# Prachet-Dev-Singh/DenseCLIP_Vit_multimodal

Hardware: AMD Instinct MI355X
Metric: images/sec (fwd+bwd) ViT-B/16 DenseCLIP @1024x2048 (higher is better)
Workload: dtype bf16

## Files before the change

denseclip_vit_multimodal_amd/_native.py:

```python
import ctypes
import os
import threading

_HERE = os.path.dirname(os.path.abspath(__file__))
LIB_PATH = os.environ.get("DCLIP_LIB", os.path.join(_HERE, "libdclip.so"))

F32, F16, BF16 = 0, 1, 2
EPI_STORE, EPI_GELU, EPI_RESIDUAL, EPI_GELU_BWD, EPI_SPLITK, EPI_STORE_SCALED = 0, 1, 2, 3, 4, 5
OPT_ATTN_FWD_WAVES, OPT_ATTN_DQ_WAVES, OPT_ATTN_DKDV_WAVES, OPT_GEMM_TILE, OPT_GEMM_TN_TILE = 0, 1, 2, 3, 4
OPT_ATTN_DKDV_QS, OPT_ATTN_FWD_KERNEL, OPT_ATTN_BWD_KERNEL, OPT_ATTN_BWD_BLOCK, OPT_GEMM_TN_COLSUM = 5, 6, 7, 8, 9
OPT_GEMM_EPI, OPT_GEMM_TAIL, OPT_ATTN_FP8_QK, OPT_ATTN_DQ_ISSUE, OPT_ATTN_DQ_ROWS = 10, 11, 12, 13, 14
OPT_ATTN_DQ_DEFER, OPT_GEMM_SCHED, OPT_GEMM_KLOOP = 15, 16, 17
OPT_ATTN_DQ_REDUCE = 18
OPT_ATTN_PREP_ORDER = 19
OPT_ATTN_DQ_DEFER = 15

_c_void_p = ctypes.c_void_p
_i32 = ctypes.c_int
_i64 = ctypes.c_int64
_f32 = ctypes.c_float

_SIGS = {
    "dclip_layernorm_fwd": [_c_void_p, _i32, _c_void_p, _c_void_p, _c_void_p, _i32, _c_void_p, _c_void_p,
                            _i64, _i64, _f32, _c_void_p],
    "dclip_layernorm_bwd": [_c_void_p, _i32, _c_void_p, _i32, _c_void_p, _c_void_p, _c_void_p, _c_void_p, _i32,
                            _c_void_p, _c_void_p, _i64, _i64, _c_void_p],
    "dclip_layernorm_bwd_res": [_c_void_p, _i32, _c_void_p, _i64, _c_void_p, _i32, _c_void_p, _c_void_p, _c_void_p,
                                _c_void_p, _c_void_p, _c_void_p, _i32, _c_void_p, _c_void_p, _c_void_p, _i64, _i64,
                                _c_void_p],
    "dclip_layernorm_bwd_ws_floats": [_i64, _i64],
    "dclip_layernorm_bwd_add": [_c_void_p, _i32, _c_void_p, _c_void_p, _c_void_p, _c_void_p, _c_void_p, _c_void_p,
                                _i32, _c_void_p, _c_void_p, _i32, _c_void_p, _c_void_p, _c_void_p, _i64, _i64,
                                _c_void_p],
    "dclip_layernorm_bwd_scaled_add": [_c_void_p, _i32, _c_void_p, _c_void_p, _c_void_p, _c_void_p, _c_void_p,
                                       _c_void_p, _c_void_p, _i32, _c_void_p, _i32, _c_void_p, _c_void_p, _c_void_p,
                                       _c_void_p, _c_void_p, _i64, _i64, _f32, _c_void_p, _i32, _c_void_p, _c_void_p],
    "dclip_gemm": [_i32, _i32, _c_void_p, _i64, _c_void_p, _i64, _i64, _i64, _i64, _i32, _f32, _c_void_p, _c_void_p,
# ... 127 lines not shown
```

denseclip_vit_multimodal_amd/_torch_ops.py:

```python
import os

import torch

_HERE = os.path.dirname(os.path.abspath(__file__))
LIB_PATH = os.environ.get("DCLIP_TORCH_LIB", os.path.join(_HERE, "libdclip_torch.so"))

_loaded = False


def load():
    global _loaded
    if _loaded:
        return torch.ops.dclip
    if not os.path.exists(LIB_PATH):
        raise RuntimeError(f"libdclip_torch.so not found at {LIB_PATH}: build it with "
                           "`make -C denseclip_vit_multimodal_amd/csrc` (the HIP path has no CPU fallback)")
    from . import _native
    bound = os.path.realpath(os.path.join(os.path.dirname(LIB_PATH), "libdclip.so"))
    if os.path.realpath(_native.LIB_PATH) != bound:
        raise RuntimeError(f"DCLIP_LIB ({_native.LIB_PATH}) is not the libdclip.so that {LIB_PATH} binds ({bound}); "
                           "build a matching adapter and point DCLIP_TORCH_LIB at it")
    _native.load()
    torch.ops.load_library(LIB_PATH)
    _register_fakes()
# ... 26 lines not shown
    def _(dy, x, w, mean, rstd, res, add, ntok, dw, db, lp_dtype):
        return _e(*x.shape, like=x, dtype=f32), _e(*x.shape, like=x, dtype=lp_dtype)

    @reg("dclip::gemm")
    def _(A, B, epi, bias, aux, out_dtype, alpha, scale=None):
        return _e(A.shape[0], B.shape[0], like=A, dtype=out_dtype)

    @reg("dclip::gemm_gelu")
    def _(A, B, bias):
        return _e(A.shape[0], B.shape[0], like=A), _e(A.shape[0], B.shape[0], like=A)

    @reg("dclip::gemm_gelu_h")
    def _(A, B, bias):
        return _e(A.shape[0], B.shape[0], like=A)

    @reg("dclip::gemm_residual_lp")
    def _(A, B, bias, aux):
        return _e(A.shape[0], B.shape[0], like=A, dtype=f32), _e(A.shape[0], B.shape[0], like=A)

    @reg("dclip::weight_grad")
    def _(dy, x, alpha, db, scale=None):
        return _e(dy.shape[1], x.shape[1], like=dy, dtype=f32)

    @reg("dclip::gemm_tn")
    def _(A, B):
        return _e(A.shape[1], B.shape[1], like=A, dtype=f32)

    @reg("dclip::cast")
    def _(x, dtype, scale, scale_t=None):
        return _e(*x.shape, like=x, dtype=dtype)

    @reg("dclip::bn_eval")
    def _(x, w, b, running_mean, running_var, eps, relu):
        return torch.empty_like(x, memory_format=torch.channels_last)

    @reg("dclip::row_scale_add")
    def _(x, y, s):
        return torch.empty_like(y)

    @reg("dclip::grad_scale")
    def _(g, target):
        return _e(4, like=g, dtype=f32)

    @reg("dclip::transpose2d")
    def _(x, dtype):
        return _e(x.shape[1], x.shape[0], like=x, dtype=dtype)
# ... 135 lines not shown
```

denseclip_vit_multimodal_amd/csrc/attention.hip:

```cpp
#include <type_traits>

#include "attn_frag.h"

namespace {

typedef int i32x4 __attribute__((ext_vector_type(4)));
template <int ROWS, int NT>
struct TileRegs {
    static constexpr int PER = ROWS * 8 / NT;
    i32x4 v[PER];
};

template <typename T, int ROWS, int NT>
__device__ __forceinline__ void tile_load(TileRegs<ROWS, NT>& R, const T* __restrict__ base, int64_t ld, int r0,
                                          int N) {
#pragma unroll
    for (int i = 0; i < TileRegs<ROWS, NT>::PER; ++i) {
        const int idx = i * NT + threadIdx.x;
        int gr = r0 + (idx >> 3);
        gr = gr < N ? gr : N - 1;
        gr = gr > 0 ? gr : 0;
        R.v[i] = *(const i32x4*)(base + (int64_t)gr * ld + (idx & 7) * 8);
    }
}
// ... 2200 lines not shown
}

template <typename T>
bool bwd2_launch(const void* qkv, const void* o, const void* dout, const float* lse, float* delta, void* dqkv, int B,
                 int N, int H, float scale, hipStream_t st, void* f8ws = nullptr) {
    if (N < 257 || dclip_option(DCLIP_OPT_ATTN_BWD_KERNEL) == 1) return false;
    const bool ragged = (N - 1) % 256 != 0;
    const int bwd_block = f8ws != nullptr ? 0 : dclip_option(DCLIP_OPT_ATTN_BWD_BLOCK);
    if (ragged && (dclip_option(DCLIP_OPT_ATTN_DQ_WAVES) == 4 ||
                   (bwd_block != 0 && bwd_block != 5 && bwd_block != 6 && bwd_block != 7 && bwd_block != 8 &&
                    bwd_block != 9 && bwd_block != 10)))
        return false;
    const int nsplit = (N + R0_CHUNK - 1) / R0_CHUNK;
    float* ws0 = delta + (int64_t)B * H * N;
    float* nstat = ws0 + (int64_t)B * H * ((N + 63) / 64) * 192;
    const bool dq4 = dclip_option(DCLIP_OPT_ATTN_DQ_WAVES) == 4;
    if ((bwd_block == 0 || bwd_block == 9 || bwd_block == 10) && f8ws == nullptr) {
        const int64_t bhn = (int64_t)B * H * N;
        float* ds0v = nstat + 2 * bhn;
        void* part = (void*)(((uintptr_t)(ds0v + bhn) + 255) & ~(uintptr_t)255);
        const int nqp = attn_bwd1_prep_blocks(N), nkb = (N - 1 + 255) / 256;
        float* r0kv = ws0;
        float* r0q = ws0 + (int64_t)B * H * nqp * 128;
        attn_bwd1_launch(std::is_same<T, bf16>::value ? DCLIP_BF16 : DCLIP_F16, qkv, o, dout, lse, delta, nstat, ds0v,
                         r0kv, r0q, part, dqkv, B, N, H, scale, st);
        attn_bwd_row0_fold_merge<T><<<B * H, 64, 0, st>>>((const T*)qkv, (const T*)dout, lse, delta, r0kv, nqp, r0q, nkb,
                                                          (T*)dqkv, N, H, scale, 1.0f / LOG2E);
        return true;
    }
    if (bwd_block == 0 || bwd_block == 6 || bwd_block == 7 || bwd_block == 8) {
        const int nq = (N - 1 + (dq4 ? 127 : 255)) / (dq4 ? 128 : 256), nkb = (N - 1 + 255) / 256;
        float* r0kv = ws0;
        float* r0q = ws0 + (int64_t)B * H * nq * 128;
        if (dq4)
            attn_bwd_dq2_kernel<T, 4><<<B * H * nq, 256, 0, st>>>((const T*)qkv, (const T*)o, (const T*)dout, lse,
                                                                   delta, nstat, (T*)dqkv, N, H, scale, r0kv);
        else if (dclip_option(DCLIP_OPT_ATTN_DQ_DEFER) == 1)
            attn_bwd_dq2_kernel<T, 8, false, 1, true><<<B * H * nq, 512, 0, st>>>((const T*)qkv, (const T*)o,
                                                                                   (const T*)dout, lse, delta, nstat,
                                                                                   (T*)dqkv, N, H, scale, r0kv);
        else if (dclip_option(DCLIP_OPT_ATTN_DQ_ROWS) == 64)
            attn_bwd_dq2_kernel<T, 4, false, 2><<<B * H * nq, 256, 0, st>>>((const T*)qkv, (const T*)o,
                                                                             (const T*)dout, lse, delta, nstat,
                                                                             (T*)dqkv, N, H, scale, r0kv);
        else if (dclip_option(DCLIP_OPT_ATTN_DQ_ISSUE) == 1)
            attn_bwd_dq2_kernel<T, 8, true><<<B * H * nq, 512, 0, st>>>((const T*)qkv, (const T*)o, (const T*)dout,
                                                                         lse, delta, nstat, (T*)dqkv, N, H, scale, r0kv);
        else
            attn_bwd_dq2_kernel<T, 8><<<B * H * nq, 512, 0, st>>>((const T*)qkv, (const T*)o, (const T*)dout, lse,
                                                                   delta, nstat, (T*)dqkv, N, H, scale, r0kv);
// ... 101 lines not shown
extern "C" int64_t dclip_attn_bwd_workspace(int B, int N, int H) {
    const int64_t two_pass = bwd_ws_two_pass(B, N, H);
    if (N >= 257) return two_pass + (int64_t)B * H * N + (attn_bwd1_part_bytes(B, N, H) + 3) / 4 + 64;
    return two_pass;
}

static bool bwd_one_pass(int N) {
    if (N < 257 || dclip_option(DCLIP_OPT_ATTN_BWD_KERNEL) == 1) return false;
    if ((N - 1) % 256 != 0 && dclip_option(DCLIP_OPT_ATTN_DQ_WAVES) == 4) return false;
    const int blk = dclip_option(DCLIP_OPT_ATTN_BWD_BLOCK);
    return blk == 0 || blk == 9 || blk == 10;
}

extern "C" int dclip_attn_bwd(int dt, const void* qkv, const void* o, const void* dout, const float* lse,
                              float* delta_ws, void* dqkv, int B, int N, int H, int D, float scale, void* stream) {
    DCLIP_HOST_CHECK(D == HD, "dclip_attn_bwd: head_dim must be 64 (got %d)", D);
    DCLIP_HOST_CHECK(dt == DCLIP_BF16 || dt == DCLIP_F16, "dclip_attn_bwd: dtype must be f16/bf16");
    DCLIP_HOST_CHECK(B > 0 && N > 0 && H > 0, "dclip_attn_bwd: empty problem");
    DCLIP_HOST_CHECK(!bwd_one_pass(N) ||
                         (1 + 64 * (int64_t)((N - 1 + 63) / 64)) * (int64_t)((N - 1 + 255) / 256) * 128 < (1ll << 32),
                     "dclip_attn_bwd: N too large for the one-pass backward's dQ partials (N = %d; "
                     "DCLIP_OPT_ATTN_BWD_BLOCK 6 selects the two-pass backward)", N);
    hipStream_t st = (hipStream_t)stream;
    if (dt == DCLIP_BF16) bwd_launch<bf16>(qkv, o, dout, lse, delta_ws, dqkv, B, N, H, scale, st);
    else bwd_launch<f16>(qkv, o, dout, lse, delta_ws, dqkv, B, N, H, scale, st);
    DCLIP_LAUNCH_CHECK();
    return 0;
}

extern "C" int64_t dclip_attn_bwd_fp8_workspace(int B, int N, int H) {
    return bwd_ws_two_pass(B, N, H) + (attn_bwd_fp8_ws_bytes(B, N, H) + 3) / 4 + 64;
}

extern "C" int dclip_attn_bwd_fp8(int dt, const void* qkv, const void* o, const void* dout, const float* lse, float* ws,
                                  void* dqkv, int B, int N, int H, int D, float scale, void* stream) {
    DCLIP_HOST_CHECK(D == HD, "dclip_attn_bwd_fp8: head_dim must be 64 (got %d)", D);
    DCLIP_HOST_CHECK(dt == DCLIP_BF16 || dt == DCLIP_F16, "dclip_attn_bwd_fp8: dtype must be f16/bf16");
    DCLIP_HOST_CHECK(B > 0 && N > 0 && H > 0, "dclip_attn_bwd_fp8: empty problem");
    DCLIP_HOST_CHECK(ws != nullptr && ((uintptr_t)ws % 16) == 0, "dclip_attn_bwd_fp8: ws (16-B aligned) required");
    DCLIP_HOST_CHECK((int64_t)((N - 1 + 63) / 64) * (8192 + 256) < (1ll << 32),
                     "dclip_attn_bwd_fp8: N too large for the fp8 image ring");
    hipStream_t st = (hipStream_t)stream;
    const int64_t w16 = bwd_ws_two_pass(B, N, H);
    void* f8 = (void*)(((uintptr_t)(ws + w16) + 255) & ~(uintptr_t)255);
    if (dt == DCLIP_BF16) bwd_launch<bf16>(qkv, o, dout, lse, ws, dqkv, B, N, H, scale, st, f8);
    else bwd_launch<f16>(qkv, o, dout, lse, ws, dqkv, B, N, H, scale, st, f8);
// ... 4 lines not shown
```

denseclip_vit_multimodal_amd/csrc/attention_bwd1.hip:

```cpp
#include "dkdv_frag.h"

namespace {

constexpr int B1_NW = 4, B1_KB = 64 * B1_NW;
typedef Dkv2Ctx<bf16, B1_NW> B1Ring;
constexpr int B1_RING = 4 * B1Ring::SLOT;
constexpr int B1_W0 = B1_RING;
constexpr int B1_SMEM = B1_W0 + B1_KB * 4;
constexpr int B1_IMG = B1_KB * 128;
static_assert(B1_SMEM + 2 * B1_IMG <= 160 * 1024, "LDS");

__device__ __forceinline__ int lane_now() {
    int l;
    asm volatile("v_mbcnt_lo_u32_b32 %0, -1, 0\n\tv_mbcnt_hi_u32_b32 %0, -1, %0" : "=v"(l));
    return l;
}

template <typename F>
__device__ __forceinline__ F to_agpr(F v) {
    F r;
    asm volatile("" : "=a"(r) : "0"(v));
    return r;
}

// ... 821 lines not shown
    for (int e = 0; e < 8; ++e) acc[e] = w * (float)kv[e];
    const T* p = dqpart + ((int64_t)bh * Np + q) * nkb * 64 + c8;
    int j = 0;
    for (; j + 8 <= nkb; j += 8) {
        t8 v[8];
#pragma unroll
        for (int u = 0; u < 8; ++u) v[u] = __builtin_nontemporal_load((const t8*)(p + (j + u) * 64));
#pragma unroll
        for (int u = 0; u < 8; ++u)
#pragma unroll
            for (int e = 0; e < 8; ++e) acc[e] += (float)v[u][e];
    }
    for (; j < nkb; ++j) {
        const t8 v = __builtin_nontemporal_load((const t8*)(p + j * 64));
#pragma unroll
        for (int e = 0; e < 8; ++e) acc[e] += (float)v[e];
    }
    t8 r;
#pragma unroll
    for (int e = 0; e < 8; ++e) r[e] = (T)(unscaled ? acc[e] * sc : acc[e]);
    *(t8*)(dqkv + ((int64_t)b * N + q) * ld + hd * HD + c8) = r;
}

constexpr int RQ_Q = 8;
constexpr int RQ_MAX_NKB = 56;
template <typename T>
__global__ __launch_bounds__(256) void attn_bwd1_dq_reduce_lds(const T* __restrict__ dqpart,
                                                               const float* __restrict__ ds0v,
                                                               const T* __restrict__ qkv, T* __restrict__ dqkv,
                                                               int N, int H, int nkb, int nrb, float sc) {
    typedef T t2 __attribute__((ext_vector_type(2)));
    typedef unsigned u32x4 __attribute__((ext_vector_type(4)));
    extern __shared__ __attribute__((aligned(16))) char rq_lds[];
    const int rb = blockIdx.x % nrb, bh = blockIdx.x / nrb, b = bh / H, hd = bh % H;
    const int q0 = 1 + rb * RQ_Q;
    const int C = H * HD;
    const int64_t ld = 3 * (int64_t)C;
    const int64_t Np = 1 + 64 * (int64_t)((N - 1 + 63) / 64);
    const int run = nkb * 128, stride = run + 128;
    const char* src = (const char*)(dqpart + ((int64_t)bh * Np + q0) * nkb * 64);
    const int chunks = RQ_Q * nkb * 8;
    for (int c = threadIdx.x; c < chunks; c += 256) {
        const int qi = c / (nkb * 8), w = c - qi * (nkb * 8);
        const u32x4 v = __builtin_nontemporal_load((const u32x4*)(src + (int64_t)c * 16));
        *(u32x4*)(rq_lds + qi * stride + w * 16) = v;
    }
// ... 1 lines not shown
    const int qi = threadIdx.x >> 5, cp = threadIdx.x & 31;
    const int q = q0 + qi;
    if (q >= N) return;
    const t2 kv = *(const t2*)(qkv + (int64_t)b * N * ld + C + hd * HD + 2 * cp);
    constexpr bool unscaled = std::is_same<T, bf16>::value;
    const float w = ds0v[(int64_t)bh * N + q] * (unscaled ? 1.0f : sc);
    float a0 = w * (float)kv[0], a1 = w * (float)kv[1];
    const char* row = rq_lds + qi * stride + cp * 4;
#pragma unroll 8
    for (int j = 0; j < nkb; ++j) {
        const t2 v = *(const t2*)(row + j * 128);
        a0 += (float)v[0];
        a1 += (float)v[1];
    }
    const t2 r = {(T)(unscaled ? a0 * sc : a0), (T)(unscaled ? a1 * sc : a1)};
    *(t2*)(dqkv + ((int64_t)b * N + q) * ld + hd * HD + 2 * cp) = r;
}

template <typename T>
void bwd1_launch(const void* qkv, const void* o, const void* dout, const float* lse, float* delta, float* nstat,
                 float* ds0v, float* r0kv, int nqp, float* r0q, void* dqpart, void* dqkv, int B, int N, int H,
                 float scale, hipStream_t st) {
    const int nkb = (N - 1 + B1_KB - 1) / B1_KB;
    attn_bwd1_prep_kernel<T><<<B * H * nqp, 256, 0, st>>>((const T*)qkv, (const T*)o, (const T*)dout, lse, delta, nstat,
                                                          ds0v, r0kv, N, H, nqp,
                                                          dclip_option(DCLIP_OPT_ATTN_PREP_ORDER) == 1);
    if (dclip_option(DCLIP_OPT_ATTN_BWD_BLOCK) != 9)
        attn_bwd1b_kernel<T><<<B * H * nkb, 256, 0, st>>>((const T*)qkv, (const T*)dout, lse, delta, nstat,
                                                          nstat + (int64_t)B * H * N, (T*)dqkv, (T*)dqpart, N, H,
                                                          1.0f / LOG2E, scale, r0q);
    else
        attn_bwd1_kernel<T><<<B * H * nkb, 256, 0, st>>>((const T*)qkv, (const T*)dout, lse, delta, nstat,
                                                         nstat + (int64_t)B * H * N, (T*)dqkv, (T*)dqpart, N, H,
                                                         1.0f / LOG2E, scale, r0q);
    if (dclip_option(DCLIP_OPT_ATTN_DQ_REDUCE) == 1 && nkb <= RQ_MAX_NKB) {
        const int nrb = (N - 1 + RQ_Q - 1) / RQ_Q;
        attn_bwd1_dq_reduce_lds<T><<<B * H * nrb, 256, RQ_Q * (nkb * 128 + 128), st>>>(
            (const T*)dqpart, ds0v, (const T*)qkv, (T*)dqkv, N, H, nkb, nrb, scale / DsScale<T>::v);
        return;
    }
    const int nrb = (N - 1 + 31) / 32;
    attn_bwd1_dq_reduce<T><<<B * H * nrb, 256, 0, st>>>((const T*)dqpart, ds0v, (const T*)qkv, (T*)dqkv, N, H, nkb, nrb,
                                                        scale / DsScale<T>::v);
}

}

int attn_bwd1_prep_blocks(int N) { return (N - 1 + 127) / 128; }

int64_t attn_bwd1_part_bytes(int B, int N, int H) {
    const int64_t nkb = (N - 1 + B1_KB - 1) / B1_KB, np = 1 + 64 * (int64_t)((N - 1 + 63) / 64);
    return (int64_t)B * H * nkb * np * 128;
}

void attn_bwd1_launch(int dt, const void* qkv, const void* o, const void* dout, const float* lse, float* delta,
                      float* nstat, float* ds0v, float* r0kv, float* r0q, void* dqpart, void* dqkv, int B, int N,
                      int H, float scale, hipStream_t st) {
    const int nqp = attn_bwd1_prep_blocks(N);
// ... 6 lines not shown
```

denseclip_vit_multimodal_amd/csrc/torch_ops.cpp:

```cpp
#include <ATen/ATen.h>
#include <c10/core/DeviceGuard.h>
#include <c10/hip/HIPStream.h>
#include <torch/library.h>

#include "../../include/dclip.h"

namespace {

using at::Tensor;

int dt_code(at::ScalarType t) {
    switch (t) {
        case at::kFloat: return DCLIP_F32;
        case at::kHalf: return DCLIP_F16;
        case at::kBFloat16: return DCLIP_BF16;
        default: TORCH_CHECK(false, "dclip: unsupported dtype ", t);
    }
    return -1;
}

void* stream_of(const Tensor& t) { return (void*)c10::hip::getCurrentHIPStream(t.device().index()).stream(); }

void check_gpu(const Tensor& t, const char* what, bool contiguous = true) {
    TORCH_CHECK(t.defined(), "dclip: ", what, " is undefined");
    TORCH_CHECK(t.is_cuda(), "dclip: ", what, " must be a GPU tensor (the MI355X path has no CPU fallback)");
    if (contiguous) TORCH_CHECK(t.is_contiguous(), "dclip: ", what, " must be contiguous");
// ... 193 lines not shown
}

Tensor weight_grad(const Tensor& dy, const Tensor& x, double alpha, c10::optional<Tensor> db,
                   const c10::optional<Tensor>& scale) {
    check_gpu(dy, "dy"); check_gpu(x, "x");
    TORCH_CHECK(dy.dim() == 2 && x.dim() == 2 && dy.size(0) == x.size(0), "weight_grad: dy (M, N), x (M, K)");
    TORCH_CHECK(dy.scalar_type() == x.scalar_type(), "weight_grad: dy and x dtypes differ (", dy.scalar_type(), " vs ",
                x.scalar_type(), ")");
    c10::DeviceGuard g(dy.device());
    const int64_t M = dy.size(0), N = dy.size(1), K = x.size(1);
    check_vec(db, N, "weight_grad db");
    int splits = 0;
    int64_t k_pad = 0;
    DCLIP_CALL(dclip_gemm_tn_plan(N, K, M, &splits, &k_pad));
    Tensor dW = at::empty({N, K}, like(dy, at::kFloat));
    Tensor ws = at::empty({(int64_t)splits * (N * K + N)}, like(dy, at::kFloat));
    DCLIP_CALL(dclip_gemm_tn(DCLIP_EPI_SPLITK, dt_code(dy.scalar_type()), dy.data_ptr(), dy.stride(0), x.data_ptr(),
                             x.stride(0), N, K, M, k_pad, splits, (float)alpha, scale_entry(scale, 1), nullptr, ws.data_ptr(),
                             dW.data_ptr(), K,
                             optr<float>(db), stream_of(dy)));
    return dW;
}

Tensor gemm_tn(const Tensor& A, const Tensor& B) {
    check_gpu(A, "A"); check_gpu(B, "B");
    TORCH_CHECK(A.dim() == 2 && B.dim() == 2 && A.size(0) == B.size(0), "gemm_tn: A (K, M), B (K, N)");
    c10::DeviceGuard g(A.device());
    const int64_t K = A.size(0), M = A.size(1), N = B.size(1);
    Tensor out = at::empty({M, N}, like(A, at::kFloat));
    DCLIP_CALL(dclip_gemm_tn(DCLIP_EPI_STORE, dt_code(A.scalar_type()), A.data_ptr(), A.stride(0), B.data_ptr(),
                             B.stride(0), M, N, K, (K + 63) / 64 * 64, 1, 1.0f, nullptr, nullptr, nullptr, out.data_ptr(), N,
                             nullptr, stream_of(A)));
    return out;
}

Tensor grad_scale(const Tensor& g, double target) {
    check_gpu(g, "g");
    TORCH_CHECK(g.scalar_type() == at::kFloat && g.is_contiguous(), "grad_scale: g must be contiguous f32");
    c10::DeviceGuard gd(g.device());
    Tensor ws = at::zeros({4}, g.options());
    DCLIP_CALL(dclip_grad_scale(ptr<float>(g), g.numel(), (float)target, ptr<float>(ws), stream_of(g)));
    return ws;
}

Tensor cast(const Tensor& x, at::ScalarType dtype, double scale, const c10::optional<Tensor>& scale_t) {
    check_gpu(x, "x");
// ... 173 lines not shown
                              (int)H, 64, (float)scale, stream_of(qkv)));
    return {o, lse};
}

std::tuple<Tensor, Tensor> attn_fwd_fp8(const Tensor& qkv, int64_t B, int64_t N, int64_t H) {
    check_gpu(qkv, "qkv");
    TORCH_CHECK(qkv.dim() == 2 && qkv.size(0) == B * N && qkv.size(1) == 3 * 64 * H, "attn_fwd_fp8: qkv (B*N, 3*H*64)");
    c10::DeviceGuard g(qkv.device());
    Tensor o = at::empty({B * N, 64 * H}, qkv.options());
    Tensor lse = at::empty({B * H * N}, like(qkv, at::kFloat));
    Tensor ws = at::empty({dclip_attn_fwd_fp8_workspace((int)B, (int)N, (int)H)}, like(qkv, at::kByte));
    DCLIP_CALL(dclip_attn_fwd_fp8(dt_code(qkv.scalar_type()), qkv.data_ptr(), o.data_ptr(), ptr<float>(lse), ws.data_ptr(),
                                  (int)B, (int)N, (int)H, 64, stream_of(qkv)));
    return {o, lse};
}

Tensor attn_bwd(const Tensor& qkv, const Tensor& o, const Tensor& dout, const Tensor& lse, int64_t B, int64_t N,
                int64_t H, double scale) {
    check_gpu(qkv, "qkv"); check_gpu(o, "o"); check_gpu(dout, "dout"); check_gpu(lse, "lse");
    TORCH_CHECK(qkv.size(0) == B * N && o.sizes() == dout.sizes() && o.size(1) == 64 * H, "attn_bwd: shapes");
    c10::DeviceGuard g(qkv.device());
    Tensor ws = at::empty({dclip_attn_bwd_workspace((int)B, (int)N, (int)H)}, like(qkv, at::kFloat));
    Tensor dqkv = at::empty_like(qkv);
    DCLIP_CALL(dclip_attn_bwd(dt_code(qkv.scalar_type()), qkv.data_ptr(), o.data_ptr(), dout.data_ptr(), ptr<float>(lse),
                              ptr<float>(ws), dqkv.data_ptr(), (int)B, (int)N, (int)H, 64, (float)scale, stream_of(qkv)));
    return dqkv;
}

Tensor attn_bwd_fp8(const Tensor& qkv, const Tensor& o, const Tensor& dout, const Tensor& lse, int64_t B, int64_t N,
                    int64_t H, double scale) {
    check_gpu(qkv, "qkv"); check_gpu(o, "o"); check_gpu(dout, "dout"); check_gpu(lse, "lse");
    TORCH_CHECK(qkv.size(0) == B * N && o.sizes() == dout.sizes() && o.size(1) == 64 * H, "attn_bwd_fp8: shapes");
    c10::DeviceGuard g(qkv.device());
    Tensor ws = at::empty({dclip_attn_bwd_fp8_workspace((int)B, (int)N, (int)H)}, like(qkv, at::kFloat));
    Tensor dqkv = at::empty_like(qkv);
    DCLIP_CALL(dclip_attn_bwd_fp8(dt_code(qkv.scalar_type()), qkv.data_ptr(), o.data_ptr(), dout.data_ptr(),
                                  ptr<float>(lse), ptr<float>(ws), dqkv.data_ptr(), (int)B, (int)N, (int)H, 64,
                                  (float)scale, stream_of(qkv)));
    return dqkv;
}

Tensor im2col(const Tensor& img, int64_t p, at::ScalarType dtype) {
    check_gpu(img, "img");
    TORCH_CHECK(img.dim() == 4, "im2col: img (B, Cin, H, W)");
    c10::DeviceGuard g(img.device());
    const int64_t B = img.size(0), Cin = img.size(1), Hin = img.size(2), Win = img.size(3);
    const int64_t k_pad = (Cin * p * p + 63) / 64 * 64;
    Tensor out = at::empty({B * (Hin / p) * (Win / p), k_pad}, like(img, dtype));
// ... 433 lines not shown
    m.impl("attn_bwd", &attn_bwd);
    m.impl("attn_bwd_fp8", &attn_bwd_fp8);
    m.impl("im2col", &im2col);
    m.impl("tokens_fwd", &tokens_fwd);
    m.impl("tokens_bwd", &tokens_bwd);
    m.impl("pos_interp", &pos_interp);
    m.impl("pos_interp_bwd", &pos_interp_bwd);
    m.impl("row_mean", &row_mean);
    m.impl("score_map", &score_map);
    m.impl("score_concat", &score_concat);
    m.impl("bilinear", &bilinear);
    m.impl("bilinear_bwd", &bilinear_bwd);
    m.impl("bn_fwd", &bn_fwd);
    m.impl("bn_bwd", &bn_bwd);
    m.impl("bn_fwd_rows", &bn_fwd_rows);
    m.impl("bn_bwd_rows", &bn_bwd_rows);
    m.impl("conv3x3", &conv3x3);
    m.impl("conv3x3_wgrad", &conv3x3_wgrad);
    m.impl("upsample_ce", &upsample_ce);
    m.impl("upsample_silog_sums", &upsample_silog_sums);
    m.impl("upsample_silog_grad", &upsample_silog_grad);
    m.impl("cityscapes_prepare", &cityscapes_prepare);
}
```

denseclip_vit_multimodal_amd/ops.py:

```python
import math
import weakref

import torch

from . import _native as N

N_ = N

_DT = {torch.float32: N.F32, torch.float16: N.F16, torch.bfloat16: N.BF16}


def _dt(t):
    try:
        return _DT[t.dtype]
    except KeyError:
        raise TypeError(f"unsupported dtype {t.dtype}") from None


def _p(t):
    return None if t is None else t.data_ptr()


def _stream():
    return torch.cuda.current_stream().cuda_stream
# ... 244 lines not shown
    return D().layernorm_bwd_scaled(dy, x, w, mean, rstd, res, dw, db, st, ds.next_use(i), FP16_GRAD_AMAX, dy_scale)


def layernorm_bwd_scaled_add(dy, x, w, mean, rstd, dw, db, res, add, ntok, add_scale, ds, i, dy_scale=None):
    st = ds.site(i, x.device)
    _check(dy, x, w, mean, rstd, dw, db, res, add, add_scale, st, dy_scale)
    e0 = _tic()
    out = D().layernorm_bwd_scaled_add(dy, x, w, mean, rstd, res, add, add_scale, ntok, dw, db, st, ds.next_use(i),
                                       FP16_GRAD_AMAX, dy_scale)
    _toc("layernorm_bwd_add", e0)
    return out


def weight_grad(dy, x, want_bias=True, alpha=1.0, db=None, scale=None):
    _check(dy, x, db, scale)
    if want_bias and db is None:
        db = torch.zeros(dy.shape[1], dtype=torch.float32, device=dy.device)
    elif not want_bias:
        db = None
    e0 = _tic()
    dW = D().weight_grad(dy, x, float(alpha), db, scale)
    _toc("gemm_wgrad", e0)
    return dW, db


def gemm_tn(A, B):
    _check(A, B)
    return D().gemm_tn(A, B)


LOG2E = 1.4426950408889634


def qkv_scale_vector(C, H, device):
    key = (C, H, str(device))
    v = _QSCALE.get(key)
    if v is None:
        v = torch.ones(3 * C, dtype=torch.float32, device=device)
        v[:C] = (C // H) ** -0.5 * LOG2E
        _QSCALE[key] = v
    return v


_QSCALE = {}


# ... 347 lines not shown
            hsb = ctx.meta[5][3] if len(ctx.meta[5]) > 3 else None
            base = _readout_grad_buffer(dmap, B, Ntok, gh, gw, C)
            if base is not None and cdt == torch.bfloat16 and dp is None and hsb is None:
                dxo, dy = D().add_readout_cast(dxo, base, Ntok, cdt, 1.0)
            elif base is not None and cdt == torch.float16 and dp is None:
                dxo, s1 = D().add_readout_amax(dxo, base, Ntok, hsb, FP16_GRAD_AMAX)
            elif base is not None:
                dr = base.float() if base.dtype != torch.float32 else base.clone()
                dr.view(B, Ntok, C)[:, 0].zero_()
                dxo = dxo + _unscale_(dr, hsb)
            else:
                dxo = dxo + _unscale_(_readout_grad_dense(dmap, B, Ntok, gh, gw, C), hsb)

        dbr = dxo if dp is None else row_scale_add(None, dxo, dp[1])
        if s1 is None:
            s1 = grad_scale(dbr, cdt)
        if dy is None:
            dy = cast(dbr, cdt, scale_t=s1)
        if ds is not None and not ds.primed[0]:
            ds.prime(0, s1)
        del dbr
        dz = gemm(dy, WEIGHTS.get(w2, cdt, transposed=True), N.EPI_GELU_BWD, aux=z)
        dW2 = db2 = dW1 = db1 = None
        if wg:
            dW2, db2 = weight_grad(dy, h, db=zb2, scale=s1)
        dy_lp = LN_DY_LP and cdt == torch.bfloat16 and s1 is None
        dy16 = LN_DY_LP_FP16 and cdt == torch.float16 and C in (512, 768, 1024)
        dxh2 = gemm(dz, WEIGHTS.get(w1, cdt, transposed=True), out_dtype=cdt if (dy_lp or dy16) else torch.float32,
                    scale=None if dy16 else s1)
        dsc1 = s1 if dy16 else None
        if wg:
            dW1, db1 = weight_grad(dz, xh2, db=zb1, scale=s1)
        del dz
        dyo = None
        if cdt == torch.bfloat16 and dp is None:
            dxm, dyo = layernorm_bwd(dxh2, xm, ln2w.detach(), mu2, rs2, dln2w, dln2b, res=dxo, lp_dtype=cdt)
            s2 = None
        elif ds is not None and ds.primed[1]:
            dxm, dyo, s2 = layernorm_bwd_scaled(dxh2, xm, ln2w.detach(), mu2, rs2, dln2w, dln2b, dxo, ds, 1, dsc1)
        else:
            dxm = layernorm_bwd(dxh2, xm, ln2w.detach(), mu2, rs2, dln2w, dln2b, res=dxo, dy_scale=dsc1)
        del dxh2
        if dyo is None:
            dab = dxm if dp is None else row_scale_add(None, dxm, dp[0])
            s2 = grad_scale(dab, cdt)
            dyo = cast(dab, cdt, scale_t=s2)
            del dab
            if ds is not None:
                ds.prime(1, s2)
        do = gemm(dyo, WEIGHTS.get(w_out, cdt, transposed=True))
        dWo = dbo = dWi = dbi = None
        if wg:
            dWo, dbo = weight_grad(dyo, o, db=zbo, scale=s2)
        del dyo
        dqkv = attn_bwd(qkv, o, do, lse, B, Ntok, H, scale, fp8=bool(fp8) and ATTN_BWD_FP8)
        del do
        dxh1 = gemm(dqkv, WEIGHTS.get(w_in, cdt, transposed=True),
                    out_dtype=cdt if (dy_lp and s2 is None) or dy16 else torch.float32, scale=None if dy16 else s2)
        dsc2 = s2 if dy16 else None
        if wg:
            dWi, dbi = weight_grad(dqkv, xh1, db=zbi, scale=s2)
        del dqkv
        lk = ctx.meta[8] if len(ctx.meta) > 8 else None
        base = None
        if lk is not None and lk.g is not None and need[0] and C in (512, 768, 1024):
            base = _readout_grad_buffer(lk.g, B, Ntok, lk.gh, lk.gw, C)
            if lk.ds is None:
                base = base if base is not None and base.dtype == torch.bfloat16 else None
            elif capturing or not (lk.ds.primed[0] and dxh1.dtype in (torch.float32, torch.float16)
                                   and x.dtype == torch.float32):
                base = None
        if base is not None:
            _stat("readout_fold")
        if base is not None and lk.ds is None:
            dxm, lk.lp = layernorm_bwd_add(dxh1, x, ln1w.detach(), mu1, rs1, dln1w, dln1b, dxm, base, Ntok,
                                           torch.bfloat16)
        elif base is not None:
            dxm, lk.lp, lk.pair = layernorm_bwd_scaled_add(dxh1, x, ln1w.detach(), mu1, rs1, dln1w, dln1b, dxm, base,
                                                           Ntok, lk.hsb, lk.ds, 0, dsc2)
        else:
            dxm = layernorm_bwd(dxh1, x, ln1w.detach(), mu1, rs1, dln1w, dln1b, res=dxm, dy_scale=dsc2)
        g = lambda i, t: t if need[i] else None
        return (dxm if need[0] else None, None, g(2, dln1w), g(3, dln1b), g(4, dWi), g(5, dbi), g(6, dWo),
                g(7, dbo), g(8, dln2w), g(9, dln2b), g(10, dW1), g(11, db1), g(12, dW2), g(13, db2))


def token_rows(m):
    if m.dim() != 4 or not m.is_cuda:
        return None
    B, C, gh, gw = m.shape
    Ntok = gh * gw + 1
    if m.stride() == (Ntok * C, 1, gw * C, C) and m.storage_offset() >= C and \
            m.untyped_storage().nbytes() >= (m.storage_offset() - C + B * Ntok * C) * m.element_size():
        return m.as_strided((B * Ntok, C), (C, 1), m.storage_offset() - C)
    return None


def _readout_grad_buffer(dmap, B, Ntok, gh, gw, C):
    if dmap.stride() == (Ntok * C, 1, gw * C, C) and dmap.storage_offset() >= C and \
            dmap.untyped_storage().nbytes() >= (dmap.storage_offset() - C + B * Ntok * C) * dmap.element_size():
        _stat("readout_zero_copy")
        return dmap.as_strided((B * Ntok, C), (C, 1), dmap.storage_offset() - C)
    return None

# ... 649 lines not shown
```

include/dclip.h:

```cpp
#ifndef DCLIP_H
#define DCLIP_H

#include <stdint.h>

#ifdef __cplusplus
extern "C" {
#endif

#define DCLIP_F32 0
#define DCLIP_F16 1
#define DCLIP_BF16 2
#define DCLIP_U8 3

#define DCLIP_OK 0
#define DCLIP_ERR_ARG (-1)
#define DCLIP_ERR_HIP (-2)

#define DCLIP_EPI_STORE 0
#define DCLIP_EPI_GELU 1
#define DCLIP_EPI_RESIDUAL 2
#define DCLIP_EPI_GELU_BWD 3
#define DCLIP_EPI_SPLITK 4
#define DCLIP_EPI_STORE_SCALED 5

const char* dclip_last_error(void);
int dclip_abi_version(void);

#define DCLIP_OPT_ATTN_FWD_WAVES 0
#define DCLIP_OPT_ATTN_DQ_WAVES 1
#define DCLIP_OPT_ATTN_DKDV_WAVES 2
#define DCLIP_OPT_GEMM_TILE 3
#define DCLIP_OPT_GEMM_TN_TILE 4
#define DCLIP_OPT_ATTN_DKDV_QS 5
#define DCLIP_OPT_ATTN_BWD_KERNEL 7
#define DCLIP_OPT_ATTN_FWD_KERNEL 6
#define DCLIP_OPT_ATTN_BWD_BLOCK 8
#define DCLIP_OPT_GEMM_TN_COLSUM 9
#define DCLIP_OPT_GEMM_EPI 10
#define DCLIP_OPT_GEMM_TAIL 11
#define DCLIP_OPT_ATTN_FP8_QK 12
#define DCLIP_OPT_ATTN_DQ_ISSUE 13
#define DCLIP_OPT_ATTN_DQ_ROWS 14
#define DCLIP_OPT_ATTN_DQ_DEFER 15
#define DCLIP_OPT_GEMM_SCHED 16
#define DCLIP_OPT_GEMM_KLOOP 17
#define DCLIP_OPT_ATTN_DQ_REDUCE 18
#define DCLIP_OPT_ATTN_PREP_ORDER 19
#define DCLIP_OPT_COUNT 20
int dclip_set_option(int id, int value);

int dclip_layernorm_fwd(const void* x, int x_dt, const float* w, const float* b,
                        void* y, int y_dt, float* mean, float* rstd,
                        int64_t rows, int64_t cols, float eps, void* stream);

int dclip_layernorm_bwd(const void* dy, int dy_dt, const void* x, int x_dt,
                        const float* w, const float* mean, const float* rstd,
                        float* dx, int accumulate, float* dw, float* db,
                        int64_t rows, int64_t cols, void* stream);
int dclip_layernorm_bwd_res(const void* dy, int dy_dt, const float* dy_scale, int64_t dy_ntok,
                            const void* x, int x_dt, const float* w, const float* mean, const float* rstd,
                            const float* res, float* dx, void* lp, int lp_dt, float* dw, float* db,
                            float* ws, int64_t rows, int64_t cols, void* stream);
int64_t dclip_layernorm_bwd_ws_floats(int64_t rows, int64_t cols);

int dclip_gemm(int epilogue, int ab_dt,
               const void* A, int64_t lda, const void* B, int64_t ldb,
               int64_t M, int64_t N, int64_t K, int splits, float alpha, const float* alpha_ptr,
               const float* bias, const void* aux, int aux_dt, int64_t ld_aux,
               void* C, int c_dt, int64_t ldc, void* C2, int64_t ldc2, void* stream);

int dclip_gemm_tn_plan(int64_t M, int64_t N, int64_t K, int* splits, int64_t* K_pad);
// ... 138 lines not shown
```

Measured before the change: 63.68.

## Overlap block backward weight-gradient GEMMs with attention backward on a side stream

```diff
diff --git a/denseclip_vit_multimodal_amd/_native.py b/denseclip_vit_multimodal_amd/_native.py
--- a/denseclip_vit_multimodal_amd/_native.py
+++ b/denseclip_vit_multimodal_amd/_native.py
@@ -13,6 +13,7 @@
 OPT_ATTN_DQ_DEFER, OPT_GEMM_SCHED, OPT_GEMM_KLOOP = 15, 16, 17
 OPT_ATTN_DQ_REDUCE = 18
 OPT_ATTN_PREP_ORDER = 19
+OPT_ATTN_BWD_PHASE = 20
 OPT_ATTN_DQ_DEFER = 15
 
 _c_void_p = ctypes.c_void_p
diff --git a/denseclip_vit_multimodal_amd/_torch_ops.py b/denseclip_vit_multimodal_amd/_torch_ops.py
--- a/denseclip_vit_multimodal_amd/_torch_ops.py
+++ b/denseclip_vit_multimodal_amd/_torch_ops.py
@@ -72,6 +72,18 @@
     def _(dy, x, alpha, db, scale=None):
         return _e(dy.shape[1], x.shape[1], like=dy, dtype=f32)
 
+    @reg("dclip_lane::weight_grad")
+    def _(dy, x, alpha, db, scale, defer):
+        return _e(dy.shape[1], x.shape[1], like=dy, dtype=f32)
+
+    @reg("dclip_lane::join")
+    def _(like):
+        return None
+
+    @reg("dclip_lane::stats")
+    def _(like):
+        return [0, 0, 0, 0]
+
     @reg("dclip::gemm_tn")
     def _(A, B):
         return _e(A.shape[1], B.shape[1], like=A, dtype=f32)
diff --git a/denseclip_vit_multimodal_amd/csrc/attention.hip b/denseclip_vit_multimodal_amd/csrc/attention.hip
--- a/denseclip_vit_multimodal_amd/csrc/attention.hip
+++ b/denseclip_vit_multimodal_amd/csrc/attention.hip
@@ -2246,10 +2246,15 @@
         const int nqp = attn_bwd1_prep_blocks(N), nkb = (N - 1 + 255) / 256;
         float* r0kv = ws0;
         float* r0q = ws0 + (int64_t)B * H * nqp * 128;
+        const int phase = dclip_option(DCLIP_OPT_ATTN_BWD_PHASE);
+        auto merge = [&]() {
+            attn_bwd_row0_fold_merge<T><<<B * H, 64, 0, st>>>((const T*)qkv, (const T*)dout, lse, delta, r0kv, nqp, r0q,
+                                                              nkb, (T*)dqkv, N, H, scale, 1.0f / LOG2E);
+        };
+        if (phase == 2) merge();
         attn_bwd1_launch(std::is_same<T, bf16>::value ? DCLIP_BF16 : DCLIP_F16, qkv, o, dout, lse, delta, nstat, ds0v,
                          r0kv, r0q, part, dqkv, B, N, H, scale, st);
-        attn_bwd_row0_fold_merge<T><<<B * H, 64, 0, st>>>((const T*)qkv, (const T*)dout, lse, delta, r0kv, nqp, r0q, nkb,
-                                                          (T*)dqkv, N, H, scale, 1.0f / LOG2E);
+        if (phase == 0) merge();
         return true;
     }
     if (bwd_block == 0 || bwd_block == 6 || bwd_block == 7 || bwd_block == 8) {
@@ -2397,6 +2402,7 @@
                      "dclip_attn_bwd: N too large for the one-pass backward's dQ partials (N = %d; "
                      "DCLIP_OPT_ATTN_BWD_BLOCK 6 selects the two-pass backward)", N);
     hipStream_t st = (hipStream_t)stream;
+    if (dclip_option(DCLIP_OPT_ATTN_BWD_PHASE) == 1 && !bwd_one_pass(N)) return 0;
     if (dt == DCLIP_BF16) bwd_launch<bf16>(qkv, o, dout, lse, delta_ws, dqkv, B, N, H, scale, st);
     else bwd_launch<f16>(qkv, o, dout, lse, delta_ws, dqkv, B, N, H, scale, st);
     DCLIP_LAUNCH_CHECK();
diff --git a/denseclip_vit_multimodal_amd/csrc/attention_bwd1.hip b/denseclip_vit_multimodal_amd/csrc/attention_bwd1.hip
--- a/denseclip_vit_multimodal_amd/csrc/attention_bwd1.hip
+++ b/denseclip_vit_multimodal_amd/csrc/attention_bwd1.hip
@@ -867,6 +867,53 @@
     *(t8*)(dqkv + ((int64_t)b * N + q) * ld + hd * HD + c8) = r;
 }
 
+template <typename T>
+__global__ __launch_bounds__(256) void attn_bwd1_dq_reduce_slim(
+    const T* __restrict__ dqpart, const float* __restrict__ ds0v, const T* __restrict__ qkv, T* __restrict__ dqkv, int N,
+    int H, int nkb, int nrb, float sc) {
+    typedef T t8 __attribute__((ext_vector_type(8)));
+    typedef unsigned u32x4 __attribute__((ext_vector_type(4)));
+    const int rb = blockIdx.x % nrb, bh = blockIdx.x / nrb, b = bh / H, hd = bh % H;
+    const int q = 1 + rb * 32 + (threadIdx.x >> 3), c8 = (threadIdx.x & 7) * 8;
+    if (q >= N) return;
+    const int C = H * HD;
+    const int64_t ld = 3 * (int64_t)C;
+    const int64_t Np = 1 + 64 * (int64_t)((N - 1 + 63) / 64);
+    const t8 kv = *(const t8*)(qkv + (int64_t)b * N * ld + C + hd * HD + c8);
+    constexpr bool unscaled = std::is_same<T, bf16>::value;
+    const float w = ds0v[(int64_t)bh * N + q] * (unscaled ? 1.0f : sc);
+    float acc[8];
+#pragma unroll
+    for (int e = 0; e < 8; ++e) acc[e] = w * (float)kv[e];
+    const T* p = dqpart + ((int64_t)bh * Np + q) * nkb * 64 + c8;
+    int j = 0;
+#pragma unroll 1
+    for (; j + 4 <= nkb; j += 4) {
+        u32x4 v[4];
+#pragma unroll
+        for (int u = 0; u < 4; ++u) v[u] = __builtin_nontemporal_load((const u32x4*)(p + (j + u) * 64));
+#pragma unroll
+        for (int u = 0; u < 4; ++u) {
+            asm volatile("" : "+v"(v[u]));
+            const t8 x = __builtin_bit_cast(t8, v[u]);
+#pragma unroll
+            for (int e = 0; e < 8; ++e) acc[e] += (float)x[e];
+            asm volatile(""
+                         : "+v"(acc[0]), "+v"(acc[1]), "+v"(acc[2]), "+v"(acc[3]), "+v"(acc[4]), "+v"(acc[5]),
+                           "+v"(acc[6]), "+v"(acc[7]));
+        }
+    }
+    for (; j < nkb; ++j) {
+        const t8 v = __builtin_nontemporal_load((const t8*)(p + j * 64));
+#pragma unroll
+        for (int e = 0; e < 8; ++e) acc[e] += (float)v[e];
+    }
+    t8 r;
+#pragma unroll
+    for (int e = 0; e < 8; ++e) r[e] = (T)(unscaled ? acc[e] * sc : acc[e]);
+    *(t8*)(dqkv + ((int64_t)b * N + q) * ld + hd * HD + c8) = r;
+}
+
 constexpr int RQ_Q = 8;
 constexpr int RQ_MAX_NKB = 56;
 template <typename T>
@@ -914,10 +961,13 @@
                  float* ds0v, float* r0kv, int nqp, float* r0q, void* dqpart, void* dqkv, int B, int N, int H,
                  float scale, hipStream_t st) {
     const int nkb = (N - 1 + B1_KB - 1) / B1_KB;
-    attn_bwd1_prep_kernel<T><<<B * H * nqp, 256, 0, st>>>((const T*)qkv, (const T*)o, (const T*)dout, lse, delta, nstat,
-                                                          ds0v, r0kv, N, H, nqp,
-                                                          dclip_option(DCLIP_OPT_ATTN_PREP_ORDER) == 1);
-    if (dclip_option(DCLIP_OPT_ATTN_BWD_BLOCK) != 9)
+    const int phase = dclip_option(DCLIP_OPT_ATTN_BWD_PHASE);
+    if (phase != 2)
+        attn_bwd1_prep_kernel<T><<<B * H * nqp, 256, 0, st>>>((const T*)qkv, (const T*)o, (const T*)dout, lse, delta,
+                                                              nstat, ds0v, r0kv, N, H, nqp,
+                                                              dclip_option(DCLIP_OPT_ATTN_PREP_ORDER) == 1);
+    if (phase == 2) {
+    } else if (dclip_option(DCLIP_OPT_ATTN_BWD_BLOCK) != 9)
         attn_bwd1b_kernel<T><<<B * H * nkb, 256, 0, st>>>((const T*)qkv, (const T*)dout, lse, delta, nstat,
                                                           nstat + (int64_t)B * H * N, (T*)dqkv, (T*)dqpart, N, H,
                                                           1.0f / LOG2E, scale, r0q);
@@ -925,7 +975,15 @@
         attn_bwd1_kernel<T><<<B * H * nkb, 256, 0, st>>>((const T*)qkv, (const T*)dout, lse, delta, nstat,
                                                          nstat + (int64_t)B * H * N, (T*)dqkv, (T*)dqpart, N, H,
                                                          1.0f / LOG2E, scale, r0q);
-    if (dclip_option(DCLIP_OPT_ATTN_DQ_REDUCE) == 1 && nkb <= RQ_MAX_NKB) {
+    if (phase == 1) return;
+    const int red = dclip_option(DCLIP_OPT_ATTN_DQ_REDUCE);
+    if (red == 2 || (red == 0 && phase == 2)) {
+        const int nrb = (N - 1 + 31) / 32;
+        attn_bwd1_dq_reduce_slim<T><<<B * H * nrb, 256, 0, st>>>((const T*)dqpart, ds0v, (const T*)qkv, (T*)dqkv, N, H,
+                                                                 nkb, nrb, scale / DsScale<T>::v);
+        return;
+    }
+    if (red == 1 && nkb <= RQ_MAX_NKB) {
         const int nrb = (N - 1 + RQ_Q - 1) / RQ_Q;
         attn_bwd1_dq_reduce_lds<T><<<B * H * nrb, 256, RQ_Q * (nkb * 128 + 128), st>>>(
             (const T*)dqpart, ds0v, (const T*)qkv, (T*)dqkv, N, H, nkb, nrb, scale / DsScale<T>::v);
diff --git a/denseclip_vit_multimodal_amd/csrc/torch_ops.cpp b/denseclip_vit_multimodal_amd/csrc/torch_ops.cpp
--- a/denseclip_vit_multimodal_amd/csrc/torch_ops.cpp
+++ b/denseclip_vit_multimodal_amd/csrc/torch_ops.cpp
@@ -1,7 +1,12 @@
 #include <ATen/ATen.h>
 #include <c10/core/DeviceGuard.h>
 #include <c10/hip/HIPStream.h>
+#include <hip/hip_runtime_api.h>
 #include <torch/library.h>
+
+#include <map>
+#include <mutex>
+#include <vector>
 
 #include "../../include/dclip.h"
 
@@ -241,6 +246,112 @@
     return dW;
 }
 
+#define HIP_OK(expr)                                                                       \
+    do {                                                                                   \
+        const hipError_t e_ = (expr);                                                      \
+        TORCH_CHECK(e_ == hipSuccess, "dclip side lane: ", #expr, ": ", hipGetErrorString(e_)); \
+    } while (0)
+
+struct SideGemm {
+    Tensor dy, x, dW, ws, db, scale;
+    int splits;
+    int64_t k_pad;
+    float alpha;
+};
+
+struct SideLane {
+    hipStream_t stream = nullptr;
+    hipEvent_t fork = nullptr, done = nullptr;
+    std::vector<SideGemm> pending;
+    std::vector<Tensor> held;
+    bool busy = false;
+    int64_t launches = 0, forks = 0, mid_forks = 0, joins = 0;
+};
+
+std::mutex g_lane_mu;
+std::map<int, SideLane> g_lanes;
+
+SideLane& lane_of(int dev) {
+    SideLane& L = g_lanes[dev];
+    if (L.stream == nullptr) {
+        L.stream = c10::hip::getStreamFromPool(false, (c10::DeviceIndex)dev).stream();
+        HIP_OK(hipEventCreateWithFlags(&L.fork, hipEventDisableTiming));
+        HIP_OK(hipEventCreateWithFlags(&L.done, hipEventDisableTiming));
+    }
+    return L;
+}
+
+void lane_fork(SideLane& L, int dev, bool mid) {
+    if (L.pending.empty()) return;
+    HIP_OK(hipEventRecord(L.fork, c10::hip::getCurrentHIPStream((c10::DeviceIndex)dev).stream()));
+    HIP_OK(hipStreamWaitEvent(L.stream, L.fork, 0));
+    std::vector<SideGemm> work;
+    work.swap(L.pending);
+    L.busy = true;
+    L.forks += 1;
+    L.mid_forks += mid;
+    for (SideGemm& g : work) {
+        for (const Tensor& t : {g.dy, g.x, g.dW, g.ws, g.db, g.scale})
+            if (t.defined()) L.held.push_back(t);
+    }
+    for (SideGemm& g : work) {
+        const int64_t N = g.dy.size(1), K = g.x.size(1), M = g.dy.size(0);
+        DCLIP_CALL(dclip_gemm_tn(DCLIP_EPI_SPLITK, dt_code(g.dy.scalar_type()), g.dy.data_ptr(), g.dy.stride(0),
+                                 g.x.data_ptr(), g.x.stride(0), N, K, M, g.k_pad, g.splits, g.alpha,
+                                 g.scale.defined() ? (const float*)g.scale.data_ptr() + 1 : nullptr, nullptr,
+                                 g.ws.data_ptr(), g.dW.data_ptr(), K, ptr<float>(g.db), (void*)L.stream));
+        L.launches += 1;
+    }
+}
+
+Tensor side_weight_grad(const Tensor& dy, const Tensor& x, double alpha, c10::optional<Tensor> db,
+                        const c10::optional<Tensor>& scale, bool defer) {
+    check_gpu(dy, "dy"); check_gpu(x, "x");
+    TORCH_CHECK(dy.dim() == 2 && x.dim() == 2 && dy.size(0) == x.size(0), "side_weight_grad: dy (M, N), x (M, K)");
+    TORCH_CHECK(dy.scalar_type() == x.scalar_type(), "side_weight_grad: dy and x dtypes differ (", dy.scalar_type(),
+                " vs ", x.scalar_type(), ")");
+    c10::DeviceGuard g(dy.device());
+    const int64_t N = dy.size(1), K = x.size(1), M = dy.size(0);
+    check_vec(db, N, "side_weight_grad db");
+    scale_entry(scale, 1);
+    SideGemm w;
+    DCLIP_CALL(dclip_gemm_tn_plan(N, K, M, &w.splits, &w.k_pad));
+    w.dy = dy; w.x = x; w.alpha = (float)alpha;
+    if (db.has_value() && db->defined()) w.db = *db;
+    if (scale.has_value() && scale->defined()) w.scale = *scale;
+    w.dW = at::empty({N, K}, like(dy, at::kFloat));
+    w.ws = at::empty({(int64_t)w.splits * (N * K + N)}, like(dy, at::kFloat));
+    Tensor out = w.dW;
+    const int dev = dy.device().index();
+    std::lock_guard<std::mutex> lk(g_lane_mu);
+    SideLane& L = lane_of(dev);
+    L.pending.push_back(std::move(w));
+    if (!defer) lane_fork(L, dev, false);
+    return out;
+}
+
+void side_join(const Tensor& like_t) {
+    check_gpu(like_t, "tensor", false);
+    c10::DeviceGuard g(like_t.device());
+    const int dev = like_t.device().index();
+    std::lock_guard<std::mutex> lk(g_lane_mu);
+    SideLane& L = lane_of(dev);
+    lane_fork(L, dev, false);
+    if (!L.busy) return;
+    HIP_OK(hipEventRecord(L.done, L.stream));
+    HIP_OK(hipStreamWaitEvent(c10::hip::getCurrentHIPStream((c10::DeviceIndex)dev).stream(), L.done, 0));
+    L.held.clear();
+    L.busy = false;
+    L.joins += 1;
+}
+
+std::vector<int64_t> side_stats(const Tensor& like_t) {
+    std::lock_guard<std::mutex> lk(g_lane_mu);
+    auto it = g_lanes.find(like_t.device().index());
+    if (it == g_lanes.end()) return {0, 0, 0, 0};
+    return {it->second.launches, it->second.forks, it->second.mid_forks, it->second.joins};
+}
+
 Tensor gemm_tn(const Tensor& A, const Tensor& B) {
     check_gpu(A, "A"); check_gpu(B, "B");
     TORCH_CHECK(A.dim() == 2 && B.dim() == 2 && A.size(0) == B.size(0), "gemm_tn: A (K, M), B (K, N)");
@@ -460,8 +571,26 @@
     c10::DeviceGuard g(qkv.device());
     Tensor ws = at::empty({dclip_attn_bwd_workspace((int)B, (int)N, (int)H)}, like(qkv, at::kFloat));
     Tensor dqkv = at::empty_like(qkv);
-    DCLIP_CALL(dclip_attn_bwd(dt_code(qkv.scalar_type()), qkv.data_ptr(), o.data_ptr(), dout.data_ptr(), ptr<float>(lse),
-                              ptr<float>(ws), dqkv.data_ptr(), (int)B, (int)N, (int)H, 64, (float)scale, stream_of(qkv)));
+    auto run = [&]() {
+        DCLIP_CALL(dclip_attn_bwd(dt_code(qkv.scalar_type()), qkv.data_ptr(), o.data_ptr(), dout.data_ptr(),
+                                  ptr<float>(lse), ptr<float>(ws), dqkv.data_ptr(), (int)B, (int)N, (int)H, 64,
+                                  (float)scale, stream_of(qkv)));
+    };
+    const int dev = qkv.device().index();
+    std::lock_guard<std::mutex> lk(g_lane_mu);
+    auto it = g_lanes.find(dev);
+    if (it == g_lanes.end() || it->second.pending.empty()) {
+        run();
+        return dqkv;
+    }
+    struct Restore {
+        ~Restore() { dclip_set_option(DCLIP_OPT_ATTN_BWD_PHASE, 0); }
+    } restore;
+    dclip_set_option(DCLIP_OPT_ATTN_BWD_PHASE, 1);
+    run();
+    lane_fork(it->second, dev, true);
+    dclip_set_option(DCLIP_OPT_ATTN_BWD_PHASE, 2);
+    run();
     return dqkv;
 }
 
@@ -941,3 +1070,15 @@
     m.impl("upsample_silog_grad", &upsample_silog_grad);
     m.impl("cityscapes_prepare", &cityscapes_prepare);
 }
+
+TORCH_LIBRARY(dclip_lane, m) {
+    m.def("weight_grad(Tensor dy, Tensor x, float alpha, Tensor(a!)? db, Tensor? scale, bool defer) -> Tensor");
+    m.def("join(Tensor like) -> ()");
+    m.def("stats(Tensor like) -> int[]");
+}
+
+TORCH_LIBRARY_IMPL(dclip_lane, CUDA, m) {
+    m.impl("weight_grad", &side_weight_grad);
+    m.impl("join", &side_join);
+    m.impl("stats", &side_stats);
+}
diff --git a/denseclip_vit_multimodal_amd/ops.py b/denseclip_vit_multimodal_amd/ops.py
--- a/denseclip_vit_multimodal_amd/ops.py
+++ b/denseclip_vit_multimodal_amd/ops.py
@@ -1,4 +1,5 @@
 import math
+import os
 import weakref
 
 import torch
@@ -290,6 +291,27 @@
     dW = D().weight_grad(dy, x, float(alpha), db, scale)
     _toc("gemm_wgrad", e0)
     return dW, db
+
+
+WGRAD_OVERLAP = int(os.environ.get("DCLIP_WGRAD_OVERLAP", "1"))
+
+
+def weight_grad_side(dy, x, db, defer):
+    _check(dy, x, db)
+    e0 = _tic()
+    D()
+    dW = torch.ops.dclip_lane.weight_grad(dy, x, 1.0, db, None, bool(defer))
+    _toc("gemm_wgrad", e0)
+    return dW, db
+
+
+def side_join(t):
+    torch.ops.dclip_lane.join(t)
+
+
+def side_stats(t):
+    D()
+    return tuple(torch.ops.dclip_lane.stats(t))
 
 
 def gemm_tn(A, B):
@@ -683,14 +705,21 @@
         del dbr
         dz = gemm(dy, WEIGHTS.get(w2, cdt, transposed=True), N.EPI_GELU_BWD, aux=z)
         dW2 = db2 = dW1 = db1 = None
-        if wg:
+        lane = (WGRAD_OVERLAP and wg and cdt == torch.bfloat16 and dp is None and s1 is None
+                and not capturing)
+        if lane:
+            _stat("wgrad_overlap")
+            dW2, db2 = weight_grad_side(dy, h, zb2, True)
+        elif wg:
             dW2, db2 = weight_grad(dy, h, db=zb2, scale=s1)
         dy_lp = LN_DY_LP and cdt == torch.bfloat16 and s1 is None
         dy16 = LN_DY_LP_FP16 and cdt == torch.float16 and C in (512, 768, 1024)
         dxh2 = gemm(dz, WEIGHTS.get(w1, cdt, transposed=True), out_dtype=cdt if (dy_lp or dy16) else torch.float32,
                     scale=None if dy16 else s1)
         dsc1 = s1 if dy16 else None
-        if wg:
+        if lane:
+            dW1, db1 = weight_grad_side(dz, xh2, zb1, True)
+        elif wg:
             dW1, db1 = weight_grad(dz, xh2, db=zb1, scale=s1)
         del dz
         dyo = None
@@ -711,7 +740,9 @@
                 ds.prime(1, s2)
         do = gemm(dyo, WEIGHTS.get(w_out, cdt, transposed=True))
         dWo = dbo = dWi = dbi = None
-        if wg:
+        if lane:
+            dWo, dbo = weight_grad_side(dyo, o, zbo, True)
+        elif wg:
             dWo, dbo = weight_grad(dyo, o, db=zbo, scale=s2)
         del dyo
         dqkv = attn_bwd(qkv, o, do, lse, B, Ntok, H, scale, fp8=bool(fp8) and ATTN_BWD_FP8)
@@ -719,7 +750,9 @@
         dxh1 = gemm(dqkv, WEIGHTS.get(w_in, cdt, transposed=True),
                     out_dtype=cdt if (dy_lp and s2 is None) or dy16 else torch.float32, scale=None if dy16 else s2)
         dsc2 = s2 if dy16 else None
-        if wg:
+        if lane and WGRAD_OVERLAP == 2:
+            dWi, dbi = weight_grad_side(dqkv, xh1, zbi, False)
+        elif wg:
             dWi, dbi = weight_grad(dqkv, xh1, db=zbi, scale=s2)
         del dqkv
         lk = ctx.meta[8] if len(ctx.meta) > 8 else None
@@ -741,6 +774,8 @@
                                                            Ntok, lk.hsb, lk.ds, 0, dsc2)
         else:
             dxm = layernorm_bwd(dxh1, x, ln1w.detach(), mu1, rs1, dln1w, dln1b, res=dxm, dy_scale=dsc2)
+        if lane:
+            side_join(x)
         g = lambda i, t: t if need[i] else None
         return (dxm if need[0] else None, None, g(2, dln1w), g(3, dln1b), g(4, dWi), g(5, dbi), g(6, dWo),
                 g(7, dbo), g(8, dln2w), g(9, dln2b), g(10, dW1), g(11, db1), g(12, dW2), g(13, db2))
diff --git a/include/dclip.h b/include/dclip.h
--- a/include/dclip.h
+++ b/include/dclip.h
@@ -46,7 +46,8 @@
 #define DCLIP_OPT_GEMM_KLOOP 17
 #define DCLIP_OPT_ATTN_DQ_REDUCE 18
 #define DCLIP_OPT_ATTN_PREP_ORDER 19
-#define DCLIP_OPT_COUNT 20
+#define DCLIP_OPT_ATTN_BWD_PHASE 20
+#define DCLIP_OPT_COUNT 21
 int dclip_set_option(int id, int value);
 
 int dclip_layernorm_fwd(const void* x, int x_dt, const float* w, const float* b,
```

Measured after the change: 64.45 (median of 6 runs). Within noise of the previous version (+1.2%).
